# TimSC/PyFeatureTrack

Measured on AMD Instinct MI355X. Metric: features tracked/sec, higher is better.
Workload: dtype f32 (convolutions accumulate in f64)

## Files before the change

include/klt_gpu.h:

```cpp
#ifndef KLT_GPU_H
#define KLT_GPU_H

#include <stdint.h>

#ifdef __cplusplus
extern "C" {
#endif

#define KLT_ABI_VERSION 11
#define KLT_MAX_KERNEL_WIDTH 71
#define KLT_MAX_LEVELS 8

typedef enum {
    KLT_OK = 0,
    KLT_ERR_ARG = -1,
    KLT_ERR_DEVICE = -2,
    KLT_ERR_STATE = -3,
    KLT_ERR_NOMEM = -4,
    KLT_ERR_TIMEOUT = -5
} klt_status;

enum { KLT_TRACKED = 0, KLT_NOT_FOUND = -1, KLT_SMALL_DET = -2, KLT_MAX_ITERATIONS = -3,
       KLT_OOB = -4, KLT_LARGE_RESIDUE = -5,
       KLT_FB_INCONSISTENT = -6,
// ... 11 lines not shown
    float   min_determinant, min_displacement, step_factor, max_residue;
    double  min_eigenvalue;
    double  grad_sigma, smooth_sigma, pyramid_sigma;
    double  borderx, bordery;
} klt_params;

typedef struct klt_ctx klt_ctx;

int         klt_abi_version(void);
int         klt_device_count(void);
int         klt_create(int device, klt_ctx **out);
void        klt_destroy(klt_ctx *ctx);
const char *klt_last_error(klt_ctx *ctx);
int         klt_sync(klt_ctx *ctx);
void       *klt_stream_handle(klt_ctx *ctx);

#define KLT_OPT_FUSED_KERNELS 1
#define KLT_OPT_SELECT_AFFINE_STATE 4
#define KLT_OPT_TOPK_PREFILTER 5
#define KLT_OPT_SELECT_PARALLEL_NMS 8
#define KLT_OPT_SAT_VARIANT 10
#define KLT_OPT_TRACK_VARIANT 11
#define KLT_OPT_FUSED_HREDUCE 12
#define KLT_OPT_TRACK_XCD_ORDER 13
#define KLT_OPT_BUILD_STREAM 15
#define KLT_OPT_TRACK_TREE_SUMS 18
#define KLT_OPT_SCORE_SETS 16
#define KLT_OPT_COPY_STREAMS 20
#define KLT_OPT_FAIL_ALLOC_AFTER 19
#define KLT_OPT_L0_STREAM 21
#define KLT_OPT_L0_LAZY_GRAD 22
#define KLT_OPT_L0_LEAN_FORM 23
#define KLT_L0_LEAN_FORM_DEFAULT 1
#define KLT_L0_LEAN_WAVE_SEG 32
int klt_set_option(klt_ctx *ctx, int option, int value);

int klt_set_params(klt_ctx *ctx, const klt_params *p);
int klt_set_kernels(klt_ctx *ctx, int which, const double *gauss, int ng, const double *deriv, int nd);

int klt_upload_u8(klt_ctx *ctx, int slot, const uint8_t *px, int ncols, int nrows, int pitch);
int klt_upload_f32(klt_ctx *ctx, int slot, const float *px, int ncols, int nrows, int pitch);
int klt_host_alloc(klt_ctx *ctx, size_t bytes, void **out);
int klt_host_free(klt_ctx *ctx, void *p);
int klt_upload_u8_async(klt_ctx *ctx, int slot, const uint8_t *px, int ncols, int nrows, int pitch);
int klt_upload_f32_async(klt_ctx *ctx, int slot, const float *px, int ncols, int nrows, int pitch);
int klt_upload_wait(klt_ctx *ctx);
int klt_host_compare(const void *a, const void *b, size_t bytes);
int klt_host_copy(void *dst, const void *src, size_t bytes);
int klt_host_lanes(void);
int klt_host_compare_rows(const uint8_t *const *rows, int nrows, size_t row_bytes, const void *b);
int klt_host_copy_rows(void *dst, const uint8_t *const *rows, int nrows, size_t row_bytes);
int klt_host_thread_serial(int on);
int klt_host_sample_rows(const uint8_t *const *rows, int nrows, int ncols, int ystep, int xstep, uint8_t *out, size_t cap);
int klt_host_luma_rows(float *dst, const uint8_t *const *rows, int nrows, int ncols);
int klt_slot_adopt_u8(klt_ctx *ctx, int slot, const uint8_t *dev_px, int ncols, int nrows, int pitch);
int klt_device_alloc(klt_ctx *ctx, size_t bytes, void **out);
int klt_device_write(klt_ctx *ctx, void *dev_dst, const void *host_src, size_t bytes);
int klt_device_free(klt_ctx *ctx, void *dev);
int klt_build_pyramids_async(klt_ctx *ctx, int slot);
int klt_build_pyramids_batch_async(klt_ctx *ctx, const int *slots, int n);
int klt_build_pyramids(klt_ctx *ctx, int slot);
#define KLT_L0_TWO_PASS 0
#define KLT_L0_TILED_LDS 1
#define KLT_L0_RB16 2
#define KLT_L0_RB32 3
#define KLT_L0_RB32_HRED 4
// ... 158 lines not shown
```

pyfeaturetrack_amd/_abi.py:

```python
import ctypes as C
import os

KLT_MAX_LEVELS = 8
KLT_OPT_L0_LEAN_FORM = 23
L0_LEAN_WAVE_COLS = 232
L0_LEAN_WAVE_SEG = 32
_HERE = os.path.dirname(os.path.abspath(__file__))
LIB_PATH = os.path.join(_HERE, "csrc", "libkltgpu.so")


class KltFeat(C.Structure):
    _fields_ = [("x", C.c_float), ("y", C.c_float), ("val", C.c_int32), ("aux", C.c_int32)]


class KltQuality(C.Structure):
    _fields_ = [("residue", C.c_float), ("ncc", C.c_float), ("min_eig", C.c_float), ("val", C.c_int32)]


class KltModelParams(C.Structure):
    _fields_ = [("mode", C.c_int32), ("ncols", C.c_int32), ("nrows", C.c_int32), ("hypotheses", C.c_int32), ("seed", C.c_uint32),
                ("min_inliers", C.c_int32), ("max_error", C.c_float), ("min_area", C.c_float)]


class KltMotionModel(C.Structure):
    _fields_ = [("nxx", C.c_double), ("nxy", C.c_double), ("ntx", C.c_double), ("nyx", C.c_double), ("nyy", C.c_double),
                ("nty", C.c_double), ("d", C.c_double), ("valid", C.c_int32), ("n_candidates", C.c_int32), ("n_inliers", C.c_int32),
                ("hypothesis", C.c_int32), ("hypothesis_inliers", C.c_int32), ("pad", C.c_int32)]


class KltEpipolarParams(C.Structure):
    _fields_ = [("mode", C.c_int32), ("ncols", C.c_int32), ("nrows", C.c_int32), ("hypotheses", C.c_int32), ("seed", C.c_uint32),
                ("min_inliers", C.c_int32), ("max_error", C.c_float)]


class KltEpipolarModel(C.Structure):
    _fields_ = [("f", C.c_double * 9), ("valid", C.c_int32), ("n_candidates", C.c_int32), ("n_inliers", C.c_int32),
                ("hypothesis", C.c_int32), ("hypothesis_inliers", C.c_int32), ("pad", C.c_int32)]


# ... 222 lines not shown
```

pyfeaturetrack_amd/csrc/api_context.hip:

```cpp
#include "klt_context.h"

thread_local hipEvent_t g_klt_stamp_start = nullptr, g_klt_stamp_stop = nullptr;

namespace kltapi {

std::string g_create_error;

int fail(klt_ctx *c, int code, const std::string &msg)
{
    if (c) c->err = msg;
    return code;
}

int drain_timers(klt_ctx *c)
{
    if (c->pending.empty()) return 0;
    HIPCHK(c, hipStreamSynchronize(c->stream));
    if (c->bstream) HIPCHK(c, hipStreamSynchronize(c->bstream));
    for (Timed &t : c->pending) {
        float ms = 0.f;
        hipEventElapsedTime(&ms, t.a, t.b);
        c->acc_ms[t.fam] += ms;
        c->acc_bytes[t.fam] += t.bytes;
        c->acc_n[t.fam]++;
// ... 290 lines not shown
    if (p->nPyramidLevels > 1 && ss != 2 && ss != 4 && ss != 8 && ss != 16 && ss != 32)
        return fail(c, KLT_ERR_ARG, "subsampling must be 2, 4, 8, 16 or 32");
    if (p->nSkippedPixels < 0 || p->max_iterations < 0) return fail(c, KLT_ERR_ARG, "negative count");
    const bool relayout = !c->have_params || c->p.nPyramidLevels != p->nPyramidLevels || c->p.subsampling != ss;
    c->p = *p;
    if (c->p.nPyramidLevels == 1 && (ss < 2)) c->p.subsampling = 2;
    c->have_params = true;
    if (relayout) {
        for (Slot &s : c->slots) s.pyr_valid = false;
        c->cfg_gen++;
    }
    return KLT_OK;
}


int klt_set_option(klt_ctx *c, int option, int value)
{
    if (!c) return KLT_ERR_ARG;
    if (option == KLT_OPT_FUSED_KERNELS) { c->use_fused = value != 0; return KLT_OK; }
    if (option == KLT_OPT_SAT_VARIANT) { c->sat_variant = value; return KLT_OK; }
    if (option == KLT_OPT_TRACK_VARIANT) { g_track_variant = value; return KLT_OK; }
    if (option == KLT_OPT_FUSED_HREDUCE) { c->fuse_hreduce = value != 0; return KLT_OK; }
    if (option == KLT_OPT_L0_STREAM) { c->l0_stream = value == 2 ? 2 : value != 0; return KLT_OK; }
    if (option == KLT_OPT_L0_LAZY_GRAD) {
        if (value < 0 || value > 2) return fail(c, KLT_ERR_ARG, "KLT_OPT_L0_LAZY_GRAD takes 0, 1 or 2");
        c->l0_lazy_grad = value;
        return KLT_OK;
    }
    if (option == KLT_OPT_L0_LEAN_FORM) {
        if (value < 0 || value > 1) return fail(c, KLT_ERR_ARG, "KLT_OPT_L0_LEAN_FORM takes 0 or 1");
        c->l0_lean_form_opt = value;
        return KLT_OK;
    }
    if (option == KLT_OPT_TRACK_XCD_ORDER) { c->track_xcd_order = value != 0; return KLT_OK; }
    if (option == KLT_OPT_BUILD_STREAM) {
        if (!value && c->bstream) HIPCHK(c, hipStreamSynchronize(c->bstream));
        if (c->build_stream_on != (value != 0)) c->last_build_on_bstream = -1;
        c->build_stream_on = value != 0;
        return KLT_OK;
    }
    if (option == KLT_OPT_SCORE_SETS) {
        if (value < 2 || value > 256) return fail(c, KLT_ERR_ARG, "KLT_OPT_SCORE_SETS takes 2..256");
        if (c->sel_job) return fail(c, KLT_ERR_STATE, "a selection is pending (it may hold one of the score sets): klt_select_finish first");
        if (int rc = sync_all(c)) return rc;
        for (size_t i = (size_t)value; i < c->pre.size(); i++) hipFree(c->pre[i].keys);
        c->pre.resize((size_t)value);
        return KLT_OK;
    }
    if (option == KLT_OPT_COPY_STREAMS) {
        if (value < 1 || value > klt_ctx::kMaxCopyStreams) return fail(c, KLT_ERR_ARG, "KLT_OPT_COPY_STREAMS takes 1..8");
        if (c->cstream) HIPCHK(c, hipStreamSynchronize(c->cstream));
        for (hipStream_t x : c->cextra) if (x) HIPCHK(c, hipStreamSynchronize(x));
        c->ncopy = value;
        return KLT_OK;
    }
    if (option == KLT_OPT_FAIL_ALLOC_AFTER) { c->fail_alloc_in = value; return KLT_OK; }
    if (option == KLT_OPT_TRACK_TREE_SUMS) { c->track_tree_sums = value != 0; return KLT_OK; }
    if (option == KLT_OPT_TOPK_PREFILTER) { c->use_topk = value != 0; return KLT_OK; }
    if (option == KLT_OPT_SELECT_PARALLEL_NMS) { c->use_mis = value != 0; return KLT_OK; }
    if (option == KLT_OPT_SELECT_AFFINE_STATE) {
        if (value >= 0 && ((size_t)value >= c->aff.size() || !c->aff[value].rec)) return fail(c, KLT_ERR_STATE, "affine state not allocated");
        c->select_aff_state = value;
        return KLT_OK;
    }
    return fail(c, KLT_ERR_ARG, "unknown option");
}
// ... 90 lines not shown
```

pyfeaturetrack_amd/csrc/api_track.hip:

```cpp
#include "klt_context.h"

template <class Entry, class Match>
static Entry *cache_find(std::vector<Entry> &v, Match match)
{
    for (Entry &e : v)
        if (match(e)) return &e;
    return nullptr;
}

template <class Entry>
static Entry *cache_place(std::vector<Entry> &v, size_t capacity)
{
    if (v.size() < capacity) {
        v.emplace_back();
        return &v.back();
    }
    Entry *lru = &v[0];
    for (Entry &e : v)
        if (e.used < lru->used) lru = &e;
    return lru;
}

namespace kltapi {

// ... 132 lines not shown
    for (int i = 0; i < nslots && capable; i++) slots[i]->lazy_read = true;
}

static int check_fb_buffers(klt_ctx *c, int fb_in, int fb_out, int fb_back)
{
    if (fb_in == fb_out || (fb_back >= 0 && (fb_back == fb_in || fb_back == fb_out)))
        return fail(c, KLT_ERR_ARG, "the forward-backward check needs fb_in, fb_out and fb_back pairwise distinct");
    if (fb_back < -1) return fail(c, KLT_ERR_ARG, "fb_back must be a feature buffer or -1");
    return 0;
}

static const char *const kGuessNotDistinct = "fb_guess must be distinct from fb_out and fb_back";
static int check_guess_buffer(klt_ctx *c, int fb_guess, int fb_out, int fb_back)
{
    return own_index(c, fb_guess, {fb_out, fb_back}, "fb_guess must be a feature buffer", kGuessNotDistinct);
}

static int guess_records(klt_ctx *c, int fb_guess, int fb_out, int fb_back, int n, const klt_feat **guess)
{
    if (!fb_holds_records(c, fb_guess, n)) return fail(c, KLT_ERR_ARG, "the guess feature buffer holds fewer records than the feature list");
    *guess = c->fbs[fb_guess].d;
    return own_records(c, fb_guess, {fb_out, fb_back}, kGuessNotDistinct);
}

static int enqueue_track(klt_ctx *c, const TrackGuessArgs &a, int npairs, int nlev, bool guess = false, bool lazy = false)
{
    const double foot = 12.0 * (c->p.window_width + 1) * (c->p.window_width + 1);
    const double foot0 = lazy ? 4.0 * 14 * 14 : foot;
    TimerScope t(c, F_TRACK, (double)npairs * a.n * (foot * 2 * (nlev - 1) + foot0 * 2 + 32), c->stream);
    if (lazy) {
        TrackLazyArgs la;
        static_cast<TrackArgsBase &>(la) = a;
        for (int i = 0; i < 4; i++) { la.kg[i] = c->gauss[2].k[i]; la.kd[i] = c->deriv[2].k[i]; }
        if (launch_track_lazy(c->stream, la)) return fail(c, KLT_ERR_STATE, "tracker launch: no lazy form for this launch");
        return 0;
    }
    if (c->lightp.mode) {
        if (launch_track_light(c->stream, a, &c->light_path)) return fail(c, KLT_ERR_ARG, "unsupported window size");
        return 0;
    }
    if (guess ? launch_track_guess(c->stream, a) : launch_track(c->stream, a)) return fail(c, KLT_ERR_ARG, "unsupported window size");
    return 0;
}

static int track_single(klt_ctx *c, int slot1, int slot2, int fb_in, int fb_out, int n, bool fb, int fb_back, bool guess = false,
                        int fb_guess = -1)
{
    if (int rc = check_ready(c)) return rc;
    if (fb || guess)
        if (int rc = refuse_with_light(c, fb ? "the forward-backward check" : "a motion prior")) return rc;
    if (n < 0) return fail(c, KLT_ERR_ARG, "negative feature count");
    if (fb)
        if (int rc = check_fb_buffers(c, fb_in, fb_out, fb_back)) return rc;
    if (guess)
        if (int rc = check_guess_buffer(c, fb_guess, fb_out, fb ? fb_back : -1)) return rc;
    HIPCHK(c, hipSetDevice(c->device));
    Slot *s1, *s2;
    const bool plain = !fb && !guess && !c->lightp.mode;
    if (int rc = check_pair(c, slot1, slot2, &s1, &s2, plain)) return rc;
    if (int rc = lists_set(c, {fb_in}, n, false)) return rc;
    FeatBuf *bo;
    if (fb && fb_back >= 0)
        if (int rc = get_fb(c, fb_back, n > 0 ? n : 1, &bo)) return rc;
    if (int rc = get_fb(c, fb_out, n > 0 ? n : 1, &bo)) return rc;
    TrackGuessArgs a;
    std::memset(&a, 0, sizeof(a));
    if (guess)
// ... 232 lines not shown
```

pyfeaturetrack_amd/csrc/klt_context.h:

```cpp
#pragma once
#include <cmath>
#include <cstdio>
#include <cstdlib>
#include <algorithm>
#include <cstring>
#include <initializer_list>
#include <memory>
#include <string>
#include <utility>
#include <vector>

#include "klt_internal.h"

struct klt_ctx;

namespace kltapi {


enum Family { F_SMOOTH_GRAD, F_PYR_REDUCE, F_GRAD, F_SMOOTH_H, F_SMOOTH_V, F_PYR_H, F_PYR_V, F_GRAD_H, F_GRAD_V, F_TRACK,
              F_SAT_ROWS, F_SAT_COLS, F_EIGEN, F_SORT, F_NMS, F_SEED, F_AFFINE, F_COUNT };
inline const char *const kFamilyName[F_COUNT] = {"smooth_grad_l0", "pyramid_reduce", "gradients", "smooth_h", "smooth_v", "pyramid_h",
                                          "pyramid_v", "gradient_h", "gradient_v", "track", "sat_rows", "sat_cols",
                                          "eigen_keys", "sort", "nms", "seed_map", "affine_check"};

// ... 105 lines not shown
    hipStream_t bstream = nullptr;
    hipStream_t work = nullptr;
    bool build_stream_on = false;
    KltComm *comm = nullptr;
    std::vector<void *> pinned;
    std::vector<void *> dev_allocs;
    std::vector<size_t> dev_alloc_bytes;
    std::vector<hipEvent_t> ring;
    size_t ring_next = 0;
    uint64_t ring_serial = 0;
    std::string err;
    klt_params p{};
    bool have_params = false;
    Taps gauss[3], deriv[3];
    bool have_taps[3] = {false, false, false};
    std::vector<Slot> slots;
    std::vector<FeatBuf> fbs;
    float *tmpA = nullptr, *tmpB = nullptr;
    size_t tmp_cap = 0;
    float *h1 = nullptr;
    size_t h1_cap = 0;
    float *cimg = nullptr;
    size_t cimg_cap = 0;
    bool fuse_hreduce = true;
    int l0_stream = 2;
    int l0_path = -1;
    bool l0_merged_grad = false;
    int l0_lazy_grad = 1;
    bool l0_lean = false;
    int l0_lean_form_opt = KLT_L0_LEAN_FORM_DEFAULT;
    int l0_lean_form = 0;
    uint64_t cfg_gen = 1;
    bool track_xcd_order = true;
    uint64_t waited_built_serial = ~0ull;
    float *sel_img = nullptr, *sel_rec = nullptr, *sat = nullptr, *valmap = nullptr;
    size_t sel_cap = 0;
    unsigned long long *keys = nullptr;
    size_t keys_cap = 0;
    uint8_t *seedmap = nullptr;
    size_t seed_cap = 0, seed_n = 0;
    uint8_t seed_stamp = 0;
    const uint8_t *mask = nullptr;
    int mask_nc = 0, mask_nr = 0;
    uint8_t *mask_own = nullptr;
    size_t mask_own_cap = 0;
    klt_select_grid sel_grid{0, 0, 0};
    int grid_path = 0;
    unsigned long long *quota_buf = nullptr;
    size_t quota_buf_cap = 0;
    uint32_t *grid = nullptr;
    size_t grid_cap = 0;
    int *nms_slots = nullptr;
    size_t nms_slots_cap = 0;
    unsigned long long *keys2 = nullptr;
    size_t keys2_cap = 0;
    unsigned *topk_hist = nullptr;
    klt_feat *fl_snapshot = nullptr;
    size_t fl_snapshot_cap = 0;
    bool track_tree_sums = false;
    bool use_topk = true;
    bool use_mis = true;
    int mis_rounds_hint = 6;
    int sat_variant = 1;
    int score_rows_path = -1, score_cols_path = -1;
    unsigned *readback = nullptr;
    float *score_override = nullptr;
// ... 248 lines not shown
```

pyfeaturetrack_amd/csrc/klt_internal.h:

```cpp
#pragma once
#include <hip/hip_runtime.h>
#include <stdint.h>

#include <string>

#include "klt_gpu.h"
#include "l0_plan.h"

struct SmoothGradArgs {
    const void *raw[KLT_MAX_BATCH];
    float *rec[KLT_MAX_BATCH];
    float *cimg[KLT_MAX_BATCH];
    Taps smooth, ggauss, gderiv;
    int ncols, nrows, R;
    short dim_c[KLT_MAX_BATCH], dim_r[KLT_MAX_BATCH];
    Taps reduce;
    float *h1[KLT_MAX_BATCH];
    int h1_nc;
};

struct PyrReduceArgs {
    const float *src[KLT_MAX_BATCH];
    float *dst[KLT_MAX_BATCH];
    Taps taps;
// ... 173 lines not shown
void launch_vconv(hipStream_t s, const float *inA, const float *inB, int ncols, int nrows, float *outA, float *outB,
                  int out_rows, int ystride, int yoff, const Taps &ta, const Taps *tb, int ostride = 1);

typedef __amdgpu_buffer_rsrc_t plane_rsrc;
__device__ __forceinline__ plane_rsrc plane_of(const void *p)
{
    return __builtin_amdgcn_make_buffer_rsrc(const_cast<void *>(p), 0, 0x7fffffff, 0x00020000);
}
__device__ __forceinline__ void plane_store(plane_rsrc r, unsigned byte_off, float v)
{
    __builtin_amdgcn_raw_buffer_store_b32(__builtin_bit_cast(unsigned, v), r, byte_off, 0, 0);
}
__device__ __forceinline__ void plane_store2(plane_rsrc r, unsigned byte_off, float2 v)
{
    typedef unsigned u32x2 __attribute__((ext_vector_type(2)));
    u32x2 w;
    w.x = __builtin_bit_cast(unsigned, v.x); w.y = __builtin_bit_cast(unsigned, v.y);
    __builtin_amdgcn_raw_buffer_store_b64(w, r, byte_off, 0, 0);
}

__device__ __forceinline__ void plane_store4(plane_rsrc r, unsigned byte_off, float2 a, float2 b)
{
    typedef unsigned u32x4 __attribute__((ext_vector_type(4)));
    u32x4 w;
    w.x = __builtin_bit_cast(unsigned, a.x); w.y = __builtin_bit_cast(unsigned, a.y);
    w.z = __builtin_bit_cast(unsigned, b.x); w.w = __builtin_bit_cast(unsigned, b.y);
    __builtin_amdgcn_raw_buffer_store_b128(w, r, byte_off, 0, 0);
}
__device__ __forceinline__ float plane_load(plane_rsrc r, unsigned byte_off)
{
    return __builtin_bit_cast(float, __builtin_amdgcn_raw_buffer_load_b32(r, byte_off, 0, 0));
}

__device__ __forceinline__ int reflect_once(int i, int n)
{
    return i < 0 ? -1 - i : i >= n ? 2 * n - 1 - i : i;
}

template <int NT>
struct TapRegs { double k[NT]; };

template <int NT, int SYM, bool ZC = false>
__device__ __forceinline__ float corr_regs(const double *c , const TapRegs<NT> &t)
{
    constexpr int H = NT / 2;
    static_assert(!ZC || SYM < 0, "centre-tap elision is for the derivative taps");
    double acc = ZC ? (c[-H] - c[H]) * t.k[0] + 0.0 : c[0] * t.k[H];
#pragma unroll
    for (int jj = ZC ? -H + 1 : -H; jj < 0; jj++) {
        const double pr = SYM > 0 ? c[jj] + c[-jj] : c[jj] - c[-jj];
        acc = acc + pr * t.k[H + jj];
    }
    return (float)acc;
}

extern int g_track_variant;
size_t pyr_reduce_lds_bytes(int ss, int ntaps);
int launch_smooth_grad(hipStream_t s, const SmoothGradArgs &a, const L0Plan &plan);
int launch_pyr_vreduce(hipStream_t s, const PyrReduceArgs &a, int batch);
int launch_pyr_reduce(hipStream_t s, const PyrReduceArgs &a, int batch);

__device__ __forceinline__ float klt_window_value(float gxx, float gxy, float gyy)
{
    const float dif = gxx - gyy;
    const float sq = dif * dif;
    const double t = (double)sq + (4.0 * (double)gxy) * (double)gxy;
    const float s = (float)sqrt(t);
    const float sum = gxx + gyy;
    const float num = sum - s;
    return (float)((double)num / 2.0);
}

__host__ __device__ __forceinline__ unsigned long long klt_pack_key_bits(uint32_t val_bits, int x, int y)
{
    return ((unsigned long long)val_bits << 32) | ((unsigned long long)x << 16) | (unsigned long long)y;
}
// ... 42 lines not shown
void launch_eigen(hipStream_t s, const SelectArgs &a);
void launch_sort_desc(hipStream_t s, unsigned long long *keys, int npow2);
void launch_topk_prefilter(hipStream_t s, const unsigned long long *keys, int n, unsigned target, unsigned *hist,
                           unsigned *info , unsigned long long *out);
int  launch_nms(hipStream_t s, const NmsArgs &a);
void launch_key_threshold(hipStream_t s, const unsigned long long *keys, int n, unsigned target, unsigned *hist, unsigned *info);
int  mis_tiles(int nx, int ny);
size_t mis_stage_bytes(int R);
void launch_mis_init(hipStream_t s, const MisArgs &a);
int  launch_mis_round(hipStream_t s, const MisArgs &a, int round);
void launch_mis_compact(hipStream_t s, const MisArgs &a, unsigned long long *out, unsigned *out_count);
int  mis_tile_capacity(int R);
void launch_zero_words(hipStream_t s, unsigned *p, size_t n);
void launch_mis_prepare(hipStream_t s, const klt_feat *fl, int nfeat, int overwrite_all, int *slots, int *nfill_out, klt_feat *snapshot,
                        unsigned *zero, size_t zero_n);
void launch_eigen_hist(hipStream_t s, const SelectArgs &a);
void launch_mask_hist(hipStream_t s, const SelectArgs &a);
void launch_mis_results(hipStream_t s, unsigned *host_out, const unsigned *rem, int look, const unsigned *info, const int *placed);
void launch_mis_place(hipStream_t s, const NmsArgs &a, const unsigned *count, unsigned *rank, const int *nfill, int bound,
                      unsigned *host_out, const unsigned *rem, int look, const unsigned *info);
void launch_unpack_candidates(hipStream_t s, const unsigned long long *keys, int n, float *val, int *x, int *y);
constexpr int KLT_QUOTA_MAX_ROUNDS = 64;
void launch_quota_live(hipStream_t s, const klt_feat *fl, int nfeat, int ncols, int nrows, const QuotaArgs &g);
void launch_quota_filter(hipStream_t s, unsigned long long *keys, const unsigned *count, int bound, const QuotaArgs &g,
                         unsigned long long *thr, int ncells, unsigned *nkept);
void launch_mis_place_quota(hipStream_t s, const NmsArgs &a, const unsigned *count, const unsigned *nkept, unsigned *rank, const int *nfill,
                            int bound, unsigned *host_out, const unsigned *rem, int look, const unsigned *info);
int  launch_nms_quota(hipStream_t s, const NmsArgs &a, const QuotaArgs &g);

void launch_track_stats(hipStream_t s, const klt_feat *in, const klt_feat *out, int n, int nlevels, unsigned long long *stats);
int launch_track(hipStream_t s, const TrackArgs &a);
int launch_track_guess(hipStream_t s, const TrackGuessArgs &a);
bool track_lazy_capable(int window, int tree_sums, int n, int npairs);
int launch_track_lazy(hipStream_t s, const TrackLazyArgs &a);
int launch_track_light(hipStream_t s, const TrackArgsBase &a, int *path);
int launch_track_quality(hipStream_t s, const QualityArgs &a);
void launch_model_gather(hipStream_t s, const ModelArgs &a);
void launch_model_score(hipStream_t s, const ModelArgs &a);
void launch_model_decide(hipStream_t s, const ModelArgs &a);
void launch_epipolar_score(hipStream_t s, const EpipolarArgs &a);
void launch_epipolar_decide(hipStream_t s, const EpipolarArgs &a);
void launch_predict_cv(hipStream_t s, const klt_feat *prev, const klt_feat *cur, klt_feat *guess, int n);
void launch_extract_patch(hipStream_t s, const float *img, int nc, int nr, float x, float y, int w, float *patch, int *bad);
void launch_track_iterate(hipStream_t s, const float *t_gx, const float *t_gy, const float *t_i, const float *i2, const float *gx2,
                          const float *gy2, int nc, int nr, int w, float x2, float y2, float step, float small, float th,
                          int max_iterations, float *res);
void launch_affine(hipStream_t s, const AffineArgs &a);
void launch_affine_reset(hipStream_t s, klt_affine_rec *rec, int n);

struct KltComm;
int  comm_unique_id(void *out128, std::string &err);
int  comm_create(int device, int nranks, int rank, const void *unique_id, KltComm **out, std::string &err);
void comm_destroy(KltComm *k);
bool comm_poisoned(const KltComm *k);
int  comm_nranks(const KltComm *k);
hipEvent_t comm_last_done(const KltComm *k);
int  comm_rank(const KltComm *k);
int  comm_allgather(KltComm *k, hipStream_t producer, const void *src, void *dst, size_t bytes, std::string &err);
int  comm_gather(KltComm *k, hipStream_t producer, const void *src, void *dst, size_t bytes, int root, std::string &err);
int  comm_gatherv(KltComm *k, hipStream_t producer, const void *src, void *dst, const size_t *counts, int root, std::string &err);
void comm_set_timeout(KltComm *k, double ms);
int  comm_sendrecv(KltComm *k, hipStream_t producer, const void *src, int to, void *dst, int from, size_t bytes, std::string &err);
int  comm_fence(KltComm *k, hipStream_t consumer, std::string &err);
int  comm_wait(KltComm *k, std::string &err);
int  comm_allreduce_max(KltComm *k, double *inout, int n, std::string &err);
```

pyfeaturetrack_amd/csrc/track_kernels.hip:

```cpp
#include <cstdlib>
#include <type_traits>

#include "klt_internal.h"
#include "track_primitives.h"

#pragma clang fp contract(off)

#ifdef KLT_TRACK_CLOCKS
__device__ long long g_tclk[256 * 32];
#define TCLK(i)                                                                                               \
    do {                                                                                                      \
        asm volatile("s_waitcnt vmcnt(0) lgkmcnt(0)" ::: "memory");                                            \
        if (threadIdx.x == 0 && blockIdx.x < 256 && (i) < 32) g_tclk[blockIdx.x * 32 + (i)] = wall_clock64();   \
    } while (0)
extern "C" int klt_debug_track_clocks(long long *out) { return (int)hipMemcpyFromSymbol(out, HIP_SYMBOL(g_tclk), sizeof(g_tclk)); }
#else
#define TCLK(i) do { } while (0)
#endif

namespace {


__device__ __forceinline__ TrackLevel exchanged(const TrackLevel &l)
{
// ... 233 lines not shown
    typedef const __attribute__((address_space(4))) char *kptr;
    kptr p = (kptr)__builtin_amdgcn_kernarg_segment_ptr() + sizeof(TrackArgsBase) + (deriv ? 4 * sizeof(double) : 0);
    asm volatile("" : "+s"(p));
#pragma unroll
    for (int i = 0; i < 7; i++) t.k[i] = i < 4 ? ((const __attribute__((address_space(4))) double *)p)[i] : 0.0;
}

__device__ __forceinline__ void lazy_records(const float *plane, int nc, int nr, int cx, int cy, bool need, float *fl, int s,
                                             f32x4 &im, f32x4 &gx, f32x4 &gy)
{
    {
        const plane_rsrc pl = plane_of(plane);
        const int x0 = need ? cx - 3 : 0, y0 = need ? cy - 3 : 0;
        const unsigned col = (unsigned)reflect_once(x0 + (s < 13 ? s : 13), nc);
#pragma unroll
        for (int h = 0; h < 2; h++) {
            float v[LZ_ROWS / 2];
#pragma unroll
            for (int r = 0; r < LZ_ROWS / 2; r++)
                v[r] = plane_load(pl, 4u * (__umul24((unsigned)reflect_once(y0 + 7 * h + r, nr), (unsigned)nc) + col));
#pragma unroll
            for (int r = 0; r < LZ_ROWS / 2; r++) fl[(7 * h + r) * LZ_PW + s] = v[r];
            wave_lds_sync();
        }
    }
    {
        TapRegs<7> kg, kd;
        lazy_taps(kg, false);
        lazy_taps(kd, true);
        const float *p = fl + (s >> 3) * LZ_PW + (s & 7);
        float *d = fl + LZ_P + s;
#pragma unroll 1
        for (int j = 0; j < LZ_ROWS / 2; j++, p += 2 * LZ_PW, d += 16) {
            double w[7];
#pragma unroll
            for (int i = 0; i < 7; i++) w[i] = (double)p[i];
            d[0] = corr_regs<7, -1>(w + 3, kd);
            d[LZ_DE] = corr_regs<7, 1>(w + 3, kg);
        }
    }
    wave_lds_sync();
    f32x4 oi, ox, oy;
    {
        const int qr = s >> 1, qh = s & 1;
        const float *d = fl + LZ_P + qr * 8 + 4 * qh;
        float o[8];
#pragma unroll 1
        for (int u = 0; u < 4; u++) {
            TapRegs<7> k;
            lazy_taps(k, u >= 2);
            const float *c = d + (u >> 1) * LZ_DE + 2 * (u & 1);
            double w0[7], w1[7];
#pragma unroll
            for (int j = 0; j < 7; j++) {
                const float2 t = *reinterpret_cast<const float2 *>(c + 8 * j);
                w0[j] = (double)t.x; w1[j] = (double)t.y;
            }
            float a0, a1;
            if (u < 2) { a0 = corr_regs<7, 1>(w0 + 3, k); a1 = corr_regs<7, 1>(w1 + 3, k); }
            else { a0 = corr_regs<7, -1>(w0 + 3, k); a1 = corr_regs<7, -1>(w1 + 3, k); }
#pragma unroll
            for (int e = 0; e < 4; e++)
                if (u == e) { o[2 * e] = a0; o[2 * e + 1] = a1; }
        }
        ox.x = o[0]; ox.y = o[1]; ox.z = o[2]; ox.w = o[3];
        oy.x = o[4]; oy.y = o[5]; oy.z = o[6]; oy.w = o[7];
        const float *c = fl + (qr + 3) * LZ_PW + 3 + 4 * qh;
        oi.x = c[0]; oi.y = c[1]; oi.z = c[2]; oi.w = c[3];
    }
    wave_lds_sync();
    if (need) { im = oi; gx = ox; gy = oy; }
}

__device__ __forceinline__ f32x4 load_plane_images(const float *plane, unsigned q)
{
    return __builtin_bit_cast(f32x4, __builtin_amdgcn_raw_buffer_load_b128(plane_of(plane), 4u * q, 0, 0));
}

constexpr int GUESS_WAVES = 8, LAZY_WAVES = 16;

template <bool BATCH, int W, int WAVES = 1, bool TREE = false, bool FB = false, bool GUESS = false>
__global__ __launch_bounds__(64, WAVES % GUESS_WAVES) void track_kernel_quad(std::conditional_t<(WAVES >= LAZY_WAVES), TrackLazyArgs, TrackKernArgs<FB, GUESS>> a)
{
    constexpr bool LAZY = WAVES >= LAZY_WAVES;
    static_assert(GUESS == (WAVES >= GUESS_WAVES && !LAZY), "instantiations with a prior carry the mark in their occupancy target");
    static_assert(!LAZY || (W == 7 && !TREE && !FB && !GUESS), "level-0 gradients on demand: the plain 7x7 kernels only");
    static_assert(W == 7 || W == 15, "quad kernels exist for 7x7 and 15x15 windows");
    static_assert(!(FB && TREE), "the forward-backward check uses the reference-order sums");
    constexpr int FPW = W == 7 ? 4 : 1;
    constexpr int LPF = 64 / FPW;
    constexpr int QPR = (W + 1) / 4;
    constexpr int w = W, n = W * W, hw = W / 2, npad = track_npad(n);
    constexpr bool REUSE = W == 7;
    static_assert((W + 1) * QPR == LPF, "one quad per lane");
    extern __shared__ __attribute__((aligned(16))) float lds[];
    const int lane = threadIdx.x, g = lane / LPF, s = lane % LPF, glead = lane - s;
    int f = FPW * blockIdx.x + g;
    if (a.order) {
        const uint32_t *ord = a.order + (BATCH ? (size_t)blockIdx.y * a.n : (size_t)0);
        const int c = blockIdx.x & 7, j = FPW * (blockIdx.x >> 3) + g, pos = c * a.order_chunk + j;
        f = (j < a.order_chunk && pos < a.n) ? (int)ord[pos] : a.n;
    }
    const TrackLevel *levels = BATCH ? a.pairs[blockIdx.y].lv : a.lv;
    const klt_feat *fin = BATCH ? a.pairs[blockIdx.y].in : a.in;
    klt_feat *fout = BATCH ? a.pairs[blockIdx.y].out : a.out;
    klt_feat *fback = nullptr;
    if constexpr (FB) fback = BATCH ? a.pairs[blockIdx.y].back : a.back;
    const bool valid = f < a.n;
    const klt_feat ft = fin[valid ? f : a.n - 1];
    const bool tracked_feature = valid && ft.val >= 0;
    float xguess = ft.x, yguess = ft.y;
    if constexpr (GUESS) {
        const klt_feat *fguess = BATCH ? a.pairs[blockIdx.y].guess : a.guess;
        if (fguess) {
            const klt_feat gs = fguess[valid ? f : a.n - 1];
            if (guess_counts(gs)) { xguess = gs.x; yguess = gs.y; }
        }
// ... 13 lines not shown
    float xstart = ft.x, ystart = ft.y;
    klt_feat fwd = ft, bwd = ft;
    int pass = 0;
    do {
        float xloc = xstart, yloc = ystart;
        for (int r = 0; r < L; r++) { xloc = xloc * a.inv_ss; yloc = yloc * a.inv_ss; }
        float xout = xloc, yout = yloc;
        if constexpr (GUESS) {
            if (pass == 0) {
                xout = xguess; yout = yguess;
                for (int r = 0; r < L; r++) { xout = xout * a.inv_ss; yout = yout * a.inv_ss; }
            }
        }
        int val = KLT_TRACKED;
        uint32_t aux = 0;
        bool alive = go;

        for (int r = L - 1; r >= 0; r--) {
            if (!__any(alive)) break;
            const TrackLevel lvf = BATCH ? load_level(levels + r) : levels[r];
            const TrackLevel lv = FB && pass ? exchanged(lvf) : lvf;
            const int nc = lv.nc, nr = lv.nr;
            if (alive) { xloc = xloc * a.ss; yloc = yloc * a.ss; xout = xout * a.ss; yout = yout * a.ss; }

            const Bilinear b1 = make_bilinear(xloc, yloc);
            const bool t_ok = b1.ix - hw >= 0 && b1.iy - hw >= 0 && b1.ix + hw + 2 <= nc && b1.iy + hw + 2 <= nr;
            const bool run = alive && t_ok;
            const unsigned q1 = run ? __umul24((unsigned)(b1.iy - hw + qr), (unsigned)nc) + (unsigned)(b1.ix - hw + 4 * qh) : 0u;
            f32x4 t_qi, t_qgx, t_qgy;
            float *const fl = lds + g * LZ_FLOATS;
            if constexpr (LAZY) {
                if (r == 0) {
                    t_qi = f32x4{0.f, 0.f, 0.f, 0.f}; t_qgx = t_qi; t_qgy = t_qi;
                    lazy_records(lv.i1, nc, nr, b1.ix - hw, b1.iy - hw, run, fl, s, t_qi, t_qgx, t_qgy);
                } else {
                    load_records(lv.i1, q1, t_qi, t_qgx, t_qgy);
                }
            } else {
                load_records(lv.i1, q1, t_qi, t_qgx, t_qgy);
            }

            int it = 0, status = KLT_OOB;
            float x2 = xout, y2 = yout;
            bool iterating = run;
            Bilinear b2;
            f32x4 s_qi = {0.f, 0.f, 0.f, 0.f}, s_qgx = s_qi, s_qgy = s_qi;
            unsigned q_held = ~0u;
            auto request_footprint = [&]() {
                const bool oob = (double)(x2 - (float)hw) < 0. || (float)nc - (x2 + (float)hw) < one_plus_eps ||
                                 (double)(y2 - (float)hw) < 0. || (float)nr - (y2 + (float)hw) < one_plus_eps;
                if (iterating && oob) { status = KLT_OOB; iterating = false; }
                b2 = make_bilinear(x2, y2);
                if (REUSE) {
                    const unsigned q = __umul24((unsigned)(b2.iy - hw + qr), (unsigned)nc) + (unsigned)(b2.ix - hw + 4 * qh);
                    if constexpr (LAZY) {
                        if (r == 0) {
                            const bool need = iterating && q != q_held;
                            if (__any(need)) lazy_records(lv.i2, nc, nr, b2.ix - hw, b2.iy - hw, need, fl, s, s_qi, s_qgx, s_qgy);
                            if (need) q_held = q;
                        } else if (iterating && q != q_held) {
                            load_records(lv.i2, q, s_qi, s_qgx, s_qgy);
                            q_held = q;
                        }
                    } else
                    if (iterating && q != q_held) {
                        load_records(lv.i2, q, s_qi, s_qgx, s_qgy);
                        q_held = q;
                    }
                } else {
                    const unsigned q = iterating ? __umul24((unsigned)(b2.iy - hw + qr), (unsigned)nc) + (unsigned)(b2.ix - hw + 4 * qh) : 0u;
                    load_records(lv.i2, q, s_qi, s_qgx, s_qgy);
                }
            };
            request_footprint();

            float t_i[4], t_gx[4], t_gy[4];
            sample_quad<QPR>(t_qi, b1, t_i);
            sample_quad<QPR>(t_qgx, b1, t_gx);
            sample_quad<QPR>(t_qgy, b1, t_gy);

            while (__any(iterating)) {
                const bool act = iterating;
                float s_i[4], s_gx[4], s_gy[4];
                sample_quad<QPR>(s_qi, b2, s_i);
                sample_quad<QPR>(s_qgx, b2, s_gx);
                sample_quad<QPR>(s_qgy, b2, s_gy);
                float tree[5] = {0.f, 0.f, 0.f, 0.f, 0.f};
    #pragma unroll
                for (int m = 0; m < 4; m++) {
                    if (qr < w && 4 * qh + m < w) {
                        const int k = k0 + m;
                        const float diff = t_i[m] - s_i[m];
                        const float sx = t_gx[m] + s_gx[m];
                        const float sy = t_gy[m] + s_gy[m];
                        if (TREE) {
                            tree[0] = tree[0] + sx * sx;
                            tree[1] = tree[1] + sx * sy;
                            tree[2] = tree[2] + sy * sy;
                            tree[3] = tree[3] + diff * sx;
                            tree[4] = tree[4] + diff * sy;
                        } else {
                            gl[k] = sx * sx;
                            gl[npad + k] = sx * sy;
                            gl[2 * npad + k] = sy * sy;
                            gl[3 * npad + k] = diff * sx;
                            gl[4 * npad + k] = diff * sy;
                        }
                    }
                }
                if (!TREE) wave_lds_sync();
                float acc = 0.f;
                if (!TREE && s < 5) acc = chain_sum<n, (W > 8), (W > 8 ? 8 : 16)>(reinterpret_cast<const float4 *>(gl + s * npad));
                if (!TREE) wave_lds_sync();
                float gxx, gxy, gyy, ex, ey;
                if (TREE) {
                    gxx = group_tree_sum<LPF>(tree[0]); gxy = group_tree_sum<LPF>(tree[1]); gyy = group_tree_sum<LPF>(tree[2]);
                    ex = group_tree_sum<LPF>(tree[3]) * a.step; ey = group_tree_sum<LPF>(tree[4]) * a.step;
                } else {
                    gxx = __shfl(acc, glead); gxy = __shfl(acc, glead + 1); gyy = __shfl(acc, glead + 2);
                    ex = __shfl(acc, glead + 3) * a.step; ey = __shfl(acc, glead + 4) * a.step;
                }
                float dx, dy;
                const bool small_det = solve_step(gxx, gxy, gyy, ex, ey, a.small, dx, dy);
                if (act && small_det) { status = KLT_SMALL_DET; iterating = false; }
                if (act && !small_det) {
                    status = KLT_TRACKED;
                    x2 = x2 + dx;
                    y2 = y2 + dy;
                    it++;
                    iterating = (fabsf(dx) >= a.th || fabsf(dy) >= a.th) && it < a.max_iterations;
                }
                if (__any(iterating)) request_footprint();
            }
            if (run) { xout = x2; yout = y2; }

            const double x2d = (double)x2, y2d = (double)y2, hwd = a.half_window;
            if (run && (x2d - hwd < 0.0 || (double)nc - (x2d + hwd) < 1.001 || y2d - hwd < 0.0 || (double)nr - (y2d + hwd) < 1.001))
                status = KLT_OOB;

            const bool need_res = run && status == KLT_TRACKED && a.use_max_residue;
            if (__any(need_res)) {
                const Bilinear br = make_bilinear(x2, y2);
                f32x4 r_qi;
                if (REUSE) {
                    const unsigned q = __umul24((unsigned)(br.iy - hw + qr), (unsigned)nc) + (unsigned)(br.ix - hw + 4 * qh);
                    r_qi = s_qi;
                    if constexpr (LAZY) {
                        if (need_res && q != q_held) r_qi = r == 0 ? load_plane_images(lv.i2, q) : load_record_images(lv.i2, q);
                    } else
                    if (need_res && q != q_held) r_qi = load_record_images(lv.i2, q);
                } else {
                    const unsigned q = need_res ? __umul24((unsigned)(br.iy - hw + qr), (unsigned)nc) + (unsigned)(br.ix - hw + 4 * qh) : 0u;
                    r_qi = load_record_images(lv.i2, q);
                }
                float s_i[4];
                sample_quad<QPR>(r_qi, br, s_i);
                float sres;
                if (TREE) {
                    float part = 0.f;
    #pragma unroll
                    for (int m = 0; m < 4; m++)
                        if (qr < w && 4 * qh + m < w) part = part + fabsf(t_i[m] - s_i[m]);
                    sres = group_tree_sum<LPF>(part);
                } else {
    #pragma unroll
// ... 254 lines not shown
}

}

void launch_extract_patch(hipStream_t s, const float *img, int nc, int nr, float x, float y, int w, float *patch, int *bad)
{
    hipLaunchKernelGGL(extract_patch_kernel, dim3(1), dim3(64), 0, s, img, nc, nr, x, y, w, patch, bad);
}

void launch_track_iterate(hipStream_t s, const float *t_gx, const float *t_gy, const float *t_i, const float *i2, const float *gx2,
                          const float *gy2, int nc, int nr, int w, float x2, float y2, float step, float small, float th,
                          int max_iterations, float *res)
{
    hipLaunchKernelGGL(track_iterate_kernel, dim3(1), dim3(64), (unsigned)track_lds_bytes(w * w), s, t_gx, t_gy, t_i, i2, gx2, gy2, nc, nr, w, x2, y2, step,
                       small, th, max_iterations, res);
}

int launch_track(hipStream_t s, const TrackArgs &a)
{
    if (a.n <= 0) return 0;
    if (a.fb) {
        if (a.pairs) return a.npairs > 0 ? launch_track_t<true, true, false>(s, a) : 0;
        return launch_track_t<false, true, false>(s, a);
    }
    if (a.pairs) return a.npairs > 0 ? launch_track_t<true, false, false>(s, a) : 0;
    return launch_track_t<false, false, false>(s, a);
}

bool track_lazy_capable(int window, int tree_sums, int n, int npairs)
{
    return track_quad7_rule(window, n, npairs) && !tree_sums && n > 0 && npairs > 0;
}

int launch_track_lazy(hipStream_t s, const TrackLazyArgs &a)
{
    const unsigned ny = a.pairs ? a.npairs : 1;
    if (!track_lazy_capable(a.window, a.tree_sums, a.n, (int)ny)) return -1;
    if (a.order && a.order_refresh)
        hipLaunchKernelGGL(track_order_kernel, dim3(ny), dim3(ORDER_T), 0, s, a.in, a.pairs ? a.pairs : nullptr, a.n, a.order);
    const dim3 gq(a.order ? 8 * ((a.order_chunk + 3) / 4) : (a.n + 3) / 4, ny), block(64);
    constexpr unsigned lds = (unsigned)(4 * sizeof(float) * (LZ_FLOATS > 5 * track_npad(49) ? LZ_FLOATS : 5 * track_npad(49)));
    if (a.pairs) klt_launch((track_kernel_quad<true, 7, 1 + LAZY_WAVES>), gq, block, lds, s, a);
    else klt_launch((track_kernel_quad<false, 7, 1 + LAZY_WAVES>), gq, block, lds, s, a);
    return 0;
}

int launch_track_guess(hipStream_t s, const TrackGuessArgs &a)
{
    if (a.n <= 0) return 0;
    if (a.fb) return a.pairs ? -1 : launch_track_t<false, true, true>(s, a);
    if (a.pairs) return a.npairs > 0 ? launch_track_t<true, false, true>(s, a) : 0;
    return launch_track_t<false, false, true>(s, a);
}
```

pyfeaturetrack_amd/csrc/track_primitives.h:

```cpp
#pragma once

#include <type_traits>

#include "klt_internal.h"

#pragma clang fp contract(off)

namespace {

struct Bilinear {
    double w00, w01, w10;
    float w11;
    int ix, iy;
};

__device__ __forceinline__ Bilinear make_bilinear(float x, float y)
{
    Bilinear b;
    b.ix = (int)x;
    b.iy = (int)y;
    const float ax = (float)((double)x - (double)b.ix);
    const float ay = (float)((double)y - (double)b.iy);
    b.w00 = (1. - (double)ax) * (1. - (double)ay);
    b.w01 = (double)ax * (1. - (double)ay);
// ... 137 lines not shown
}

__device__ __forceinline__ f32x4 load_record_images(const float *rec, unsigned q)
{
    const __amdgpu_buffer_rsrc_t r = __builtin_amdgcn_make_buffer_rsrc((void *)rec, 0, 0x7fffffff, 0x00020000);
    const unsigned o = 12u * q;
    f32x4 im;
    im.x = __builtin_bit_cast(float, __builtin_amdgcn_raw_buffer_load_b32(r, o, 0, 0));
    im.y = __builtin_bit_cast(float, __builtin_amdgcn_raw_buffer_load_b32(r, o + 12u, 0, 0));
    im.z = __builtin_bit_cast(float, __builtin_amdgcn_raw_buffer_load_b32(r, o + 24u, 0, 0));
    im.w = __builtin_bit_cast(float, __builtin_amdgcn_raw_buffer_load_b32(r, o + 36u, 0, 0));
    return im;
}

template <int QPR>
__device__ __forceinline__ void sample_quad(const f32x4 a, const Bilinear &b, float out[4])
{
    f32x4 lo;
    lo.x = __shfl_down(a.x, QPR); lo.y = __shfl_down(a.y, QPR); lo.z = __shfl_down(a.z, QPR); lo.w = __shfl_down(a.w, QPR);
    const float rx = __shfl_down(a.x, 1), dx = __shfl_down(a.x, QPR + 1);
    const float v00[4] = {a.x, a.y, a.z, a.w}, v01[4] = {a.y, a.z, a.w, rx};
    const float v10[4] = {lo.x, lo.y, lo.z, lo.w}, v11[4] = {lo.y, lo.z, lo.w, dx};
#pragma unroll
    for (int m = 0; m < 4; m++) {
        const float t4 = b.w11 * v11[m];
        double d = b.w00 * (double)v00[m];
        d = d + b.w01 * (double)v01[m];
        d = d + b.w10 * (double)v10[m];
        d = d + (double)t4;
        out[m] = (float)d;
    }
}

template <class F>
inline void for_window_class(int window, F &&f)
{
    using std::integral_constant;
    const int n = window * window;
    if (window == 7) f(integral_constant<int, 1>{}, integral_constant<int, 7>{});
    else if (window == 15) f(integral_constant<int, 4>{}, integral_constant<int, 15>{});
    else if (n <= 64) f(integral_constant<int, 1>{}, integral_constant<int, 0>{});
    else if (n <= 128) f(integral_constant<int, 2>{}, integral_constant<int, 0>{});
    else if (n <= 256) f(integral_constant<int, 4>{}, integral_constant<int, 0>{});
    else if (n <= 512) f(integral_constant<int, 8>{}, integral_constant<int, 0>{});
    else f(integral_constant<int, 16>{}, integral_constant<int, 0>{});
}

}
```

Measured before the change: 250.4 million.

## Fuse first-iteration lazy gradient builds for both images into one LDS pass

Adds a new lazy-form tracker variant, on by default, for the first iteration at level 0. It loads the 14x14 patches of both the template and target images into LDS with buffer-to-LDS loads and computes the separable gradients for both together, replacing two separate per-image lazy_records passes. The row and column convolution helpers are factored into shared templates so several outputs can be produced from one staged window. The cost is more LDS per block and a different occupancy bound, and the old path stays available behind a new option.

```diff
diff --git a/include/klt_gpu.h b/include/klt_gpu.h
--- a/include/klt_gpu.h
+++ b/include/klt_gpu.h
@@ -67,6 +67,8 @@
 #define KLT_OPT_L0_LAZY_GRAD 22
 #define KLT_OPT_L0_LEAN_FORM 23
 #define KLT_L0_LEAN_FORM_DEFAULT 1
+#define KLT_OPT_TRACK_LAZY_FORM 24
+#define KLT_TRACK_LAZY_FORM_DEFAULT 1
 #define KLT_L0_LEAN_WAVE_SEG 32
 int klt_set_option(klt_ctx *ctx, int option, int value);
 
diff --git a/pyfeaturetrack_amd/_abi.py b/pyfeaturetrack_amd/_abi.py
--- a/pyfeaturetrack_amd/_abi.py
+++ b/pyfeaturetrack_amd/_abi.py
@@ -5,6 +5,7 @@
 KLT_OPT_L0_LEAN_FORM = 23
 L0_LEAN_WAVE_COLS = 232
 L0_LEAN_WAVE_SEG = 32
+KLT_OPT_TRACK_LAZY_FORM = 24
 _HERE = os.path.dirname(os.path.abspath(__file__))
 LIB_PATH = os.path.join(_HERE, "csrc", "libkltgpu.so")
 
diff --git a/pyfeaturetrack_amd/csrc/api_context.hip b/pyfeaturetrack_amd/csrc/api_context.hip
--- a/pyfeaturetrack_amd/csrc/api_context.hip
+++ b/pyfeaturetrack_amd/csrc/api_context.hip
@@ -346,6 +346,11 @@
         c->l0_lean_form_opt = value;
         return KLT_OK;
     }
+    if (option == KLT_OPT_TRACK_LAZY_FORM) {
+        if (value < 0 || value > 1) return fail(c, KLT_ERR_ARG, "KLT_OPT_TRACK_LAZY_FORM takes 0 or 1");
+        c->track_lazy_form = value;
+        return KLT_OK;
+    }
     if (option == KLT_OPT_TRACK_XCD_ORDER) { c->track_xcd_order = value != 0; return KLT_OK; }
     if (option == KLT_OPT_BUILD_STREAM) {
         if (!value && c->bstream) HIPCHK(c, hipStreamSynchronize(c->bstream));
diff --git a/pyfeaturetrack_amd/csrc/api_track.hip b/pyfeaturetrack_amd/csrc/api_track.hip
--- a/pyfeaturetrack_amd/csrc/api_track.hip
+++ b/pyfeaturetrack_amd/csrc/api_track.hip
@@ -188,7 +188,7 @@
         TrackLazyArgs la;
         static_cast<TrackArgsBase &>(la) = a;
         for (int i = 0; i < 4; i++) { la.kg[i] = c->gauss[2].k[i]; la.kd[i] = c->deriv[2].k[i]; }
-        if (launch_track_lazy(c->stream, la)) return fail(c, KLT_ERR_STATE, "tracker launch: no lazy form for this launch");
+        if (launch_track_lazy(c->stream, la, c->track_lazy_form)) return fail(c, KLT_ERR_STATE, "tracker launch: no lazy form for this launch");
         return 0;
     }
     if (c->lightp.mode) {
diff --git a/pyfeaturetrack_amd/csrc/klt_context.h b/pyfeaturetrack_amd/csrc/klt_context.h
--- a/pyfeaturetrack_amd/csrc/klt_context.h
+++ b/pyfeaturetrack_amd/csrc/klt_context.h
@@ -161,6 +161,7 @@
     int l0_lean_form = 0;
     uint64_t cfg_gen = 1;
     bool track_xcd_order = true;
+    int track_lazy_form = KLT_TRACK_LAZY_FORM_DEFAULT;
     uint64_t waited_built_serial = ~0ull;
     float *sel_img = nullptr, *sel_rec = nullptr, *sat = nullptr, *valmap = nullptr;
     size_t sel_cap = 0;
diff --git a/pyfeaturetrack_amd/csrc/klt_internal.h b/pyfeaturetrack_amd/csrc/klt_internal.h
--- a/pyfeaturetrack_amd/csrc/klt_internal.h
+++ b/pyfeaturetrack_amd/csrc/klt_internal.h
@@ -229,7 +229,7 @@
     return __builtin_bit_cast(float, __builtin_amdgcn_raw_buffer_load_b32(r, byte_off, 0, 0));
 }
 
-__device__ __forceinline__ int reflect_once(int i, int n)
+__host__ __device__ __forceinline__ int reflect_once(int i, int n)
 {
     return i < 0 ? -1 - i : i >= n ? 2 * n - 1 - i : i;
 }
@@ -238,7 +238,7 @@
 struct TapRegs { double k[NT]; };
 
 template <int NT, int SYM, bool ZC = false>
-__device__ __forceinline__ float corr_regs(const double *c , const TapRegs<NT> &t)
+__host__ __device__ __forceinline__ float corr_regs(const double *c , const TapRegs<NT> &t)
 {
     constexpr int H = NT / 2;
     static_assert(!ZC || SYM < 0, "centre-tap elision is for the derivative taps");
@@ -347,7 +347,7 @@
 int launch_track(hipStream_t s, const TrackArgs &a);
 int launch_track_guess(hipStream_t s, const TrackGuessArgs &a);
 bool track_lazy_capable(int window, int tree_sums, int n, int npairs);
-int launch_track_lazy(hipStream_t s, const TrackLazyArgs &a);
+int launch_track_lazy(hipStream_t s, const TrackLazyArgs &a, int form);
 int launch_track_light(hipStream_t s, const TrackArgsBase &a, int *path);
 int launch_track_quality(hipStream_t s, const QualityArgs &a);
 void launch_model_gather(hipStream_t s, const ModelArgs &a);
diff --git a/pyfeaturetrack_amd/csrc/track_kernels.hip b/pyfeaturetrack_amd/csrc/track_kernels.hip
--- a/pyfeaturetrack_amd/csrc/track_kernels.hip
+++ b/pyfeaturetrack_amd/csrc/track_kernels.hip
@@ -289,11 +289,10 @@
         float *d = fl + LZ_P + s;
 #pragma unroll 1
         for (int j = 0; j < LZ_ROWS / 2; j++, p += 2 * LZ_PW, d += 16) {
-            double w[7];
-#pragma unroll
-            for (int i = 0; i < 7; i++) w[i] = (double)p[i];
-            d[0] = corr_regs<7, -1>(w + 3, kd);
-            d[LZ_DE] = corr_regs<7, 1>(w + 3, kg);
+            float dd, ee;
+            lazy_row_h<1>(p, kg, kd, &dd, &ee);
+            d[0] = dd;
+            d[LZ_DE] = ee;
         }
     }
     wave_lds_sync();
@@ -307,15 +306,15 @@
             TapRegs<7> k;
             lazy_taps(k, u >= 2);
             const float *c = d + (u >> 1) * LZ_DE + 2 * (u & 1);
-            double w0[7], w1[7];
+            float c0[7], c1[7];
 #pragma unroll
             for (int j = 0; j < 7; j++) {
                 const float2 t = *reinterpret_cast<const float2 *>(c + 8 * j);
-                w0[j] = (double)t.x; w1[j] = (double)t.y;
+                c0[j] = t.x; c1[j] = t.y;
             }
             float a0, a1;
-            if (u < 2) { a0 = corr_regs<7, 1>(w0 + 3, k); a1 = corr_regs<7, 1>(w1 + 3, k); }
-            else { a0 = corr_regs<7, -1>(w0 + 3, k); a1 = corr_regs<7, -1>(w1 + 3, k); }
+            if (u < 2) { lazy_col_v<1, 1>(c0, k, &a0); lazy_col_v<1, 1>(c1, k, &a1); }
+            else { lazy_col_v<-1, 1>(c0, k, &a0); lazy_col_v<-1, 1>(c1, k, &a1); }
 #pragma unroll
             for (int e = 0; e < 4; e++)
                 if (u == e) { o[2 * e] = a0; o[2 * e + 1] = a1; }
@@ -329,17 +328,97 @@
     if (need) { im = oi; gx = ox; gy = oy; }
 }
 
+constexpr int LZE_STRIDE = 72, LZE_PATCH = 2 * LZ_ROWS * LZE_STRIDE, LZE_FLOATS = LZE_PATCH + 2 * 4 * 64;
+
+__device__ __forceinline__ void lazy_records_entry(const float *plane1, const float *plane2, int nc, int nr, int cx1, int cy1, bool need1,
+                                                   int cx2, int cy2, bool need2, float *lds, int g, int s,
+                                                   f32x4 &t_im, f32x4 &t_gx, f32x4 &t_gy, f32x4 &s_im, f32x4 &s_gx, f32x4 &s_gy)
+{
+    typedef __attribute__((address_space(3))) float *lds_ptr;
+    asm volatile("" : "+v"(s), "+v"(g));
+    auto reflect = [](int i, int n) { const int a = i ^ (i >> 31); return min(a, 2 * n - 1 - a); };
+    const int sc = s < 13 ? s : 13;
+    lds_ptr dst = (lds_ptr)lds;
+    asm volatile("" : "+s"(dst));
+    const int xa = need1 ? cx1 - 3 : 0, ya = need1 ? cy1 - 3 : 0, xb = need2 ? cx2 - 3 : 0, yb = need2 ? cy2 - 3 : 0;
+    const plane_rsrc pa = plane_of(plane1), pb = plane_of(plane2);
+    if (__all(min(min(xa, ya), min(xb, yb)) >= 0 && max(xa, xb) + LZ_ROWS <= nc && max(ya, yb) + LZ_ROWS <= nr)) {
+        const unsigned oa = 4u * (__umul24((unsigned)ya, (unsigned)nc) + (unsigned)(xa + sc));
+        const unsigned ob = 4u * (__umul24((unsigned)yb, (unsigned)nc) + (unsigned)(xb + sc));
+#pragma unroll
+        for (int r = 0; r < LZ_ROWS; r++) {
+            __builtin_amdgcn_raw_ptr_buffer_load_lds(pa, dst + r * LZE_STRIDE, 4, oa, 4 * r * nc, 0, 0);
+            __builtin_amdgcn_raw_ptr_buffer_load_lds(pb, dst + (LZ_ROWS + r) * LZE_STRIDE, 4, ob, 4 * r * nc, 0, 0);
+        }
+    } else {
+        const unsigned ca = (unsigned)reflect(xa + sc, nc), cb = (unsigned)reflect(xb + sc, nc);
+#pragma unroll
+        for (int r = 0; r < LZ_ROWS; r++) {
+            __builtin_amdgcn_raw_ptr_buffer_load_lds(pa, dst + r * LZE_STRIDE, 4,
+                                                     4u * (__umul24((unsigned)reflect(ya + r, nr), (unsigned)nc) + ca), 0, 0, 0);
+            __builtin_amdgcn_raw_ptr_buffer_load_lds(pb, dst + (LZ_ROWS + r) * LZE_STRIDE, 4,
+                                                     4u * (__umul24((unsigned)reflect(yb + r, nr), (unsigned)nc) + cb), 0, 0, 0);
+        }
+    }
+    asm volatile("s_waitcnt vmcnt(0)" ::: "memory");
+    float *const fb = lds + 16 * g;
+    const int qr = s >> 1, qh = s & 1;
+    float *const im = lds + LZE_PATCH + 64 * g;
+    if (s < LZ_ROWS) {
+        float4 *row = reinterpret_cast<float4 *>(fb + s * LZE_STRIDE);
+        float4 *keep = reinterpret_cast<float4 *>(im + 8 * (s - 3));
+        TapRegs<7> kg, kd;
+        lazy_taps(kg, false);
+        lazy_taps(kd, true);
+#pragma unroll
+        for (int p = 0; p < 2; p++, row += LZ_ROWS * LZE_STRIDE / 4, keep += 64) {
+            const float4 v0 = row[0], v1 = row[1], v2 = row[2], v3 = row[3];
+            const float v[16] = {v0.x, v0.y, v0.z, v0.w, v1.x, v1.y, v1.z, v1.w, v2.x, v2.y, v2.z, v2.w, v3.x, v3.y, v3.z, v3.w};
+            if (s >= 3 && s < 11) { keep[0] = make_float4(v[3], v[4], v[5], v[6]); keep[1] = make_float4(v[7], v[8], v[9], v[10]); }
+            float d[8], e[8];
+            lazy_row_h<8>(v, kg, kd, d, e);
+            row[0] = make_float4(d[0], d[1], d[2], d[3]); row[1] = make_float4(d[4], d[5], d[6], d[7]);
+            row[2] = make_float4(e[0], e[1], e[2], e[3]); row[3] = make_float4(e[4], e[5], e[6], e[7]);
+        }
+    }
+    wave_lds_sync();
+    {
+        float *col = fb + (s >> 3) * LZ_ROWS * LZE_STRIDE + (s & 7);
+#pragma unroll
+        for (int pl = 0; pl < 2; pl++, col += 8) {
+            TapRegs<7> k;
+            lazy_taps(k, pl);
+            float c[LZ_ROWS], out[8];
+#pragma unroll
+            for (int j = 0; j < LZ_ROWS; j++) c[j] = col[j * LZE_STRIDE];
+            if (pl) lazy_col_v<-1, 8>(c, k, out);
+            else lazy_col_v<1, 8>(c, k, out);
+#pragma unroll
+            for (int j = 0; j < 8; j++) col[j * LZE_STRIDE] = out[j];
+        }
+    }
+    wave_lds_sync();
+    const float *qd = fb + qr * LZE_STRIDE + 4 * qh;
+    const f32x4 i1 = *reinterpret_cast<const f32x4 *>(im + 4 * s), i2 = *reinterpret_cast<const f32x4 *>(im + 256 + 4 * s);
+    const f32x4 x1 = *reinterpret_cast<const f32x4 *>(qd), y1 = *reinterpret_cast<const f32x4 *>(qd + 8);
+    const f32x4 x2 = *reinterpret_cast<const f32x4 *>(qd + LZ_ROWS * LZE_STRIDE), y2 = *reinterpret_cast<const f32x4 *>(qd + LZ_ROWS * LZE_STRIDE + 8);
+    wave_lds_sync();
+    if (need1) { t_im = i1; t_gx = x1; t_gy = y1; }
+    if (need2) { s_im = i2; s_gx = x2; s_gy = y2; }
+}
+
 __device__ __forceinline__ f32x4 load_plane_images(const float *plane, unsigned q)
 {
     return __builtin_bit_cast(f32x4, __builtin_amdgcn_raw_buffer_load_b128(plane_of(plane), 4u * q, 0, 0));
 }
 
-constexpr int GUESS_WAVES = 8, LAZY_WAVES = 16;
+constexpr int GUESS_WAVES = 8, LAZY_WAVES = 16, ENTRY_WAVES = 32;
 
 template <bool BATCH, int W, int WAVES = 1, bool TREE = false, bool FB = false, bool GUESS = false>
-__global__ __launch_bounds__(64, WAVES % GUESS_WAVES) void track_kernel_quad(std::conditional_t<(WAVES >= LAZY_WAVES), TrackLazyArgs, TrackKernArgs<FB, GUESS>> a)
+__global__ __launch_bounds__(64, WAVES >= ENTRY_WAVES ? 4 : WAVES % GUESS_WAVES) void track_kernel_quad(std::conditional_t<(WAVES >= LAZY_WAVES), TrackLazyArgs, TrackKernArgs<FB, GUESS>> a)
 {
     constexpr bool LAZY = WAVES >= LAZY_WAVES;
+    constexpr bool ENTRY = WAVES >= ENTRY_WAVES;
     static_assert(GUESS == (WAVES >= GUESS_WAVES && !LAZY), "instantiations with a prior carry the mark in their occupancy target");
     static_assert(!LAZY || (W == 7 && !TREE && !FB && !GUESS), "level-0 gradients on demand: the plain 7x7 kernels only");
     static_assert(W == 7 || W == 15, "quad kernels exist for 7x7 and 15x15 windows");
@@ -419,7 +498,7 @@
             if constexpr (LAZY) {
                 if (r == 0) {
                     t_qi = f32x4{0.f, 0.f, 0.f, 0.f}; t_qgx = t_qi; t_qgy = t_qi;
-                    lazy_records(lv.i1, nc, nr, b1.ix - hw, b1.iy - hw, run, fl, s, t_qi, t_qgx, t_qgy);
+                    if constexpr (!ENTRY) lazy_records(lv.i1, nc, nr, b1.ix - hw, b1.iy - hw, run, fl, s, t_qi, t_qgx, t_qgy);
                 } else {
                     load_records(lv.i1, q1, t_qi, t_qgx, t_qgy);
                 }
@@ -433,7 +512,7 @@
             Bilinear b2;
             f32x4 s_qi = {0.f, 0.f, 0.f, 0.f}, s_qgx = s_qi, s_qgy = s_qi;
             unsigned q_held = ~0u;
-            auto request_footprint = [&]() {
+            auto request_footprint = [&](auto first) {
                 const bool oob = (double)(x2 - (float)hw) < 0. || (float)nc - (x2 + (float)hw) < one_plus_eps ||
                                  (double)(y2 - (float)hw) < 0. || (float)nr - (y2 + (float)hw) < one_plus_eps;
                 if (iterating && oob) { status = KLT_OOB; iterating = false; }
@@ -443,7 +522,13 @@
                     if constexpr (LAZY) {
                         if (r == 0) {
                             const bool need = iterating && q != q_held;
-                            if (__any(need)) lazy_records(lv.i2, nc, nr, b2.ix - hw, b2.iy - hw, need, fl, s, s_qi, s_qgx, s_qgy);
+                            if constexpr (ENTRY && decltype(first)::value) {
+                                lazy_records_entry(lv.i1, lv.i2, nc, nr, b1.ix - hw, b1.iy - hw, run, b2.ix - hw, b2.iy - hw, need, lds, g, s,
+                                                   t_qi, t_qgx, t_qgy, s_qi, s_qgx, s_qgy);
+                                float xa = x2;
+                                asm volatile("" : "+v"(xa));
+                                b2 = make_bilinear(xa, y2);
+                            } else if (__any(need)) lazy_records(lv.i2, nc, nr, b2.ix - hw, b2.iy - hw, need, fl, s, s_qi, s_qgx, s_qgy);
                             if (need) q_held = q;
                         } else if (iterating && q != q_held) {
                             load_records(lv.i2, q, s_qi, s_qgx, s_qgy);
@@ -459,7 +544,7 @@
                     load_records(lv.i2, q, s_qi, s_qgx, s_qgy);
                 }
             };
-            request_footprint();
+            request_footprint(std::true_type{});
 
             float t_i[4], t_gx[4], t_gy[4];
             sample_quad<QPR>(t_qi, b1, t_i);
@@ -517,7 +602,7 @@
                     it++;
                     iterating = (fabsf(dx) >= a.th || fabsf(dy) >= a.th) && it < a.max_iterations;
                 }
-                if (__any(iterating)) request_footprint();
+                if (__any(iterating)) request_footprint(std::false_type{});
             }
             if (run) { xout = x2; yout = y2; }
 
@@ -838,7 +923,7 @@
     return track_quad7_rule(window, n, npairs) && !tree_sums && n > 0 && npairs > 0;
 }
 
-int launch_track_lazy(hipStream_t s, const TrackLazyArgs &a)
+int launch_track_lazy(hipStream_t s, const TrackLazyArgs &a, int form)
 {
     const unsigned ny = a.pairs ? a.npairs : 1;
     if (!track_lazy_capable(a.window, a.tree_sums, a.n, (int)ny)) return -1;
@@ -846,6 +931,13 @@
         hipLaunchKernelGGL(track_order_kernel, dim3(ny), dim3(ORDER_T), 0, s, a.in, a.pairs ? a.pairs : nullptr, a.n, a.order);
     const dim3 gq(a.order ? 8 * ((a.order_chunk + 3) / 4) : (a.n + 3) / 4, ny), block(64);
     constexpr unsigned lds = (unsigned)(4 * sizeof(float) * (LZ_FLOATS > 5 * track_npad(49) ? LZ_FLOATS : 5 * track_npad(49)));
+    if (form) {
+        constexpr unsigned lds_entry = (unsigned)(sizeof(float) * LZE_FLOATS);
+        static_assert(lds_entry >= lds && lds_entry <= 10240, "sixteen wavefronts per CU");
+        if (a.pairs) klt_launch((track_kernel_quad<true, 7, 1 + LAZY_WAVES + ENTRY_WAVES>), gq, block, lds_entry, s, a);
+        else klt_launch((track_kernel_quad<false, 7, 1 + LAZY_WAVES + ENTRY_WAVES>), gq, block, lds_entry, s, a);
+        return 0;
+    }
     if (a.pairs) klt_launch((track_kernel_quad<true, 7, 1 + LAZY_WAVES>), gq, block, lds, s, a);
     else klt_launch((track_kernel_quad<false, 7, 1 + LAZY_WAVES>), gq, block, lds, s, a);
     return 0;
diff --git a/pyfeaturetrack_amd/csrc/track_primitives.h b/pyfeaturetrack_amd/csrc/track_primitives.h
--- a/pyfeaturetrack_amd/csrc/track_primitives.h
+++ b/pyfeaturetrack_amd/csrc/track_primitives.h
@@ -193,6 +193,29 @@
     }
 }
 
+template <int NOUT>
+__host__ __device__ __forceinline__ void lazy_row_h(const float *p, const TapRegs<7> &kg, const TapRegs<7> &kd, float *d, float *e)
+{
+    double w[NOUT + 6];
+#pragma unroll
+    for (int i = 0; i < NOUT + 6; i++) w[i] = (double)p[i];
+#pragma unroll
+    for (int j = 0; j < NOUT; j++) {
+        d[j] = corr_regs<7, -1>(w + 3 + j, kd);
+        e[j] = corr_regs<7, 1>(w + 3 + j, kg);
+    }
+}
+
+template <int SYM, int NOUT>
+__host__ __device__ __forceinline__ void lazy_col_v(const float *c, const TapRegs<7> &k, float *out)
+{
+    double w[NOUT + 6];
+#pragma unroll
+    for (int j = 0; j < NOUT + 6; j++) w[j] = (double)c[j];
+#pragma unroll
+    for (int j = 0; j < NOUT; j++) out[j] = corr_regs<7, SYM>(w + 3 + j, k);
+}
+
 template <class F>
 inline void for_window_class(int window, F &&f)
 {
```

Result: faster. 263.0 million (median of 6 runs) (+5.1%).
